# mandt-lab/shallow-ntc

Hardware: AMD Instinct MI355X
Metric: decode Mpixels/s + (bpp, PSNR) on Kodak, two_layer_syn (higher is better)
Workload: dtype f32

## Files before the change

include/sntc.h:

```cpp
#ifndef SNTC_H_
#define SNTC_H_

#include <stddef.h>
#include <stdint.h>

#ifdef __cplusplus
extern "C" {
#endif

#define SNTC_VERSION 100

enum {
  SNTC_OK = 0,
  SNTC_ERR_BAD_SHAPE = 1,
  SNTC_ERR_UNSUPPORTED = 2,
  SNTC_ERR_HIP = 3,
  SNTC_ERR_NONFINITE = 4,
  SNTC_ERR_NO_DEVICE = 5
};

const char* sntc_last_error(void);
int sntc_version(void);
int sntc_device_count(void);
int sntc_device_arch(int device, char* buf, size_t buflen);
// ... 80 lines not shown
int sntc_upsmall_plan_update(sntc_upsmall_plan* plan, const float* w, const float* bias, void* stream);
void sntc_upsmall_plan_destroy(sntc_upsmall_plan* plan);
int64_t sntc_upsmall_flops(const sntc_upsmall_plan* plan, int n, int h, int w);
int sntc_upsmall_forward(const sntc_upsmall_plan* plan, const float* x, int n, int h, int w, float* y, void* stream);
typedef struct sntc_syn_plan sntc_syn_plan;
typedef struct sntc_syn_batch {
  const float* y_hat;
  float* hidden;
  int32_t n, h, w;
  int32_t reserved;
} sntc_syn_batch;
int sntc_syn_supported(int k, int stride, int cin, int ch, int has_res);
int sntc_syn_plan_create(int k, int stride, int cin, int ch, int has_res, int act_kind, const float* w1, const float* b1,
                         const float* beta, const float* gamma, void* stream, sntc_syn_plan** plan);
int sntc_syn_plan_update(sntc_syn_plan* plan, const float* w1, const float* b1, const float* beta, const float* gamma, void* stream);
void sntc_syn_plan_destroy(sntc_syn_plan* plan);
int64_t sntc_syn_flops(const sntc_syn_plan* plan, int64_t latent_pixels);
int64_t sntc_syn_workspace_bytes(const sntc_syn_plan* plan);
int sntc_syn_forward(const sntc_syn_plan* plan, const sntc_syn_batch* batches, int nbatches, void* workspace, size_t workspace_bytes,
                     void* stream);
int sntc_syn_plan_set_workgroups(sntc_syn_plan* plan, int max_workgroups);
int sntc_syn_plan_units(const sntc_syn_plan* plan, int* out, int capacity);
int sntc_syn_describe(int k, int stride, int cin, int ch, int has_res, int* out, int capacity);
int sntc_syn_selfcheck(int k, int stride, int cin, int ch, int has_res, int h, int w, unsigned seed, double* max_err);
int sntc_conv_plan_set_tile(sntc_conv_plan* plan, int variant);
int sntc_conv_plan_set_schedule(sntc_conv_plan* plan, int flags);
int sntc_split3(const float* x, int64_t npix, int c, void* out, void* stream);
int sntc_dequant_split3(const int32_t* symbols, const float* hyper, int64_t npix, int c, void* out, float* y_hat,
                        void* stream);
int sntc_conv_status(int* flags, void* stream);
int sntc_conv_status_inject(int flags, void* stream);
int sntc_conv_set_stream_k(int enabled);
int sntc_conv_get_stream_k(void);
int sntc_conv_launch_info(const sntc_conv_plan* plan, int n, int h, int w, int* variant, int* nblocks);
int sntc_conv_launch_order(const sntc_conv_plan* plan, int n, int h, int w, int* column_major);
int64_t sntc_conv_tune_workspace_bytes(const sntc_conv_plan* plan, int n, int h, int w);
int sntc_conv_plan_tune(sntc_conv_plan* plan, const float* x, int n, int h, int w, float* y, const float* res,
                        const float* aux, void* workspace, size_t workspace_bytes, int reps, int* variant, int* stream_k,
                        void* stream);
int sntc_conv_plan_candidates(const sntc_conv_plan* plan, int n, int h, int w, int* variants, int* stream_k, int capacity);
int sntc_conv_plan_set_choice(sntc_conv_plan* plan, int n, int h, int w, int variant, int stream_k);
int sntc_conv_plan_clear_tuning(sntc_conv_plan* plan);
int sntc_conv_plan_drop_choice(sntc_conv_plan* plan, int n, int h, int w, int ncols);

int sntc_conv_columns_supported(const sntc_conv_plan* plan, int ncols);
int sntc_conv_forward_columns(const sntc_conv_plan* plan, const float* x, int n, int h, int w, float* y, const float* res,
                              const float* aux, void* workspace, size_t workspace_bytes, void* stream, int ncols);
int sntc_conv_forward_columns_dequant(const sntc_conv_plan* plan, const float* x, int n, int h, int w, int ncols,
                                      const int32_t* symbols, float* y_hat, void* workspace, size_t workspace_bytes, void* stream);
int64_t sntc_conv_columns_flops(const sntc_conv_plan* plan, int n, int h, int w, int ncols);
int64_t sntc_conv_columns_workspace_bytes(const sntc_conv_plan* plan, int n, int h, int w, int ncols);
int sntc_conv_columns_launch_info(const sntc_conv_plan* plan, int n, int h, int w, int ncols, int* variant, int* nblocks,
                                  int* column_major);
int64_t sntc_conv_columns_tune_workspace_bytes(const sntc_conv_plan* plan, int n, int h, int w, int ncols);
int sntc_conv_columns_tune(sntc_conv_plan* plan, const float* x, int n, int h, int w, int ncols, float* y, void* workspace,
                           size_t workspace_bytes, int reps, int* variant, int* stream_k, void* stream);
int sntc_conv_columns_candidates(const sntc_conv_plan* plan, int n, int h, int w, int ncols, int* variants, int* stream_k,
                                 int capacity);
int sntc_conv_columns_set_choice(sntc_conv_plan* plan, int n, int h, int w, int ncols, int variant, int stream_k);

int sntc_gdn_small(const float* x, int64_t npix, int c, const float* beta, const float* gamma,
                   int inverse, int alpha, int epsilon_is_half, float* y, void* stream);

int sntc_two_layer_tail(const float* t, int n, int hh, int wh, int ch, int has_res, int act_kind,
                        const float* beta, const float* gamma, const float* w2, const float* b2,
                        int k2, int s2, int cout, float* x_hat, void* stream);
// ... 198 lines not shown
```

shallow-ntc_amd/_capi.py:

```python
from __future__ import annotations

import ctypes as C
import os
from pathlib import Path

_PKG = Path(__file__).resolve().parent
LIB_PATH = Path(os.environ.get("SNTC_LIB", _PKG / "lib" / "libsntc_hip.so"))

OK, ERR_BAD_SHAPE, ERR_UNSUPPORTED, ERR_HIP, ERR_NONFINITE, ERR_NO_DEVICE = range(6)

CONV2D, CONV2D_TRANSPOSE, SIGNAL_DOWN, SIGNAL_UP = range(4)
ACT_NONE, ACT_RELU, ACT_LEAKY_RELU, ACT_SIGMOID = range(4)
PRO_NONE, PRO_ABS, PRO_SQUARE = range(3)
EPI_STORE, EPI_ADD, EPI_GATE, EPI_RES_DIV, EPI_RES_MUL, EPI_RES_DIV_SQRT, EPI_RES_MUL_SQRT, EPI_MASK_RELU, EPI_MASK_LEAKY = range(9)


class SntcError(RuntimeError):
    def __init__(self, code, msg):
        super().__init__(f"sntc error {code}: {msg}")
        self.code = code


class NonFiniteError(SntcError, ValueError):
    """Mirrors tf.debugging.check_numerics' InvalidArgumentError (reference mshyper/models.py:308-309,356)."""
# ... 37 lines not shown
    "sntc_resblock_forward": (C.c_int, [_P, _P, C.c_int, C.c_int, C.c_int, _P, _P]),
    "sntc_resblock_plan_set_workgroups": (C.c_int, [_P, C.c_int]),
    "sntc_upsmall_supported": (C.c_int, [C.c_int, C.c_int, C.c_int, C.c_int, C.c_int]),
    "sntc_upsmall_plan_create": (C.c_int, [C.c_int, C.c_int, C.c_int, C.c_int, C.c_int, _P, _P, _P, C.POINTER(_P)]),
    "sntc_upsmall_plan_update": (C.c_int, [_P, _P, _P, _P]),
    "sntc_upsmall_plan_destroy": (None, [_P]),
    "sntc_upsmall_flops": (C.c_int64, [_P, C.c_int, C.c_int, C.c_int]),
    "sntc_upsmall_forward": (C.c_int, [_P, _P, C.c_int, C.c_int, C.c_int, _P, _P]),
    "sntc_rgbconv_supported": (C.c_int, [C.c_int, C.c_int, C.c_int, C.c_int, C.c_int, C.c_int]),
    "sntc_rgbconv_plan_create": (C.c_int, [C.c_int, C.c_int, C.c_int, C.c_int, C.c_int, _P, _P, C.c_int, _P, C.POINTER(_P)]),
    "sntc_rgbconv_plan_update": (C.c_int, [_P, _P, _P, _P]),
    "sntc_rgbconv_plan_destroy": (None, [_P]),
    "sntc_rgbconv_flops": (C.c_int64, [_P, C.c_int, C.c_int, C.c_int]),
    "sntc_rgbconv_forward": (C.c_int, [_P, _P, C.c_int, C.c_int, C.c_int, _P, _P]),
    "sntc_rgbconv_plan_set_workgroups": (C.c_int, [_P, C.c_int]),
    "sntc_syn_supported": (C.c_int, [C.c_int, C.c_int, C.c_int, C.c_int, C.c_int]),
    "sntc_syn_plan_create": (C.c_int, [C.c_int, C.c_int, C.c_int, C.c_int, C.c_int, C.c_int, _P, _P, _P, _P, _P, C.POINTER(_P)]),
    "sntc_syn_plan_update": (C.c_int, [_P, _P, _P, _P, _P, _P]),
    "sntc_syn_plan_destroy": (None, [_P]),
    "sntc_syn_flops": (C.c_int64, [_P, C.c_int64]),
    "sntc_syn_workspace_bytes": (C.c_int64, [_P]),
    "sntc_syn_forward": (C.c_int, [_P, _P, C.c_int, _P, C.c_size_t, _P]),
    "sntc_syn_plan_set_workgroups": (C.c_int, [_P, C.c_int]),
    "sntc_syn_plan_units": (C.c_int, [_P, C.POINTER(C.c_int), C.c_int]),
    "sntc_syn_describe": (C.c_int, [C.c_int, C.c_int, C.c_int, C.c_int, C.c_int, C.POINTER(C.c_int), C.c_int]),
    "sntc_syn_selfcheck": (C.c_int, [C.c_int, C.c_int, C.c_int, C.c_int, C.c_int, C.c_int, C.c_int, C.c_uint, C.POINTER(C.c_double)]),
    "sntc_conv_plan_set_tile": (C.c_int, [C.c_void_p, C.c_int]),
    "sntc_conv_plan_set_schedule": (C.c_int, [C.c_void_p, C.c_int]),
    "sntc_split3": (C.c_int, [_P, C.c_int64, C.c_int, _P, _P]),
    "sntc_dequant_split3": (C.c_int, [_P, _P, C.c_int64, C.c_int, _P, _P, _P]),
    "sntc_conv_status": (C.c_int, [C.POINTER(C.c_int), _P]),
    "sntc_conv_status_inject": (C.c_int, [C.c_int, _P]),
    "sntc_conv_set_stream_k": (C.c_int, [C.c_int]),
    "sntc_conv_get_stream_k": (C.c_int, []),
    "sntc_conv_launch_info": (C.c_int, [_P, C.c_int, C.c_int, C.c_int, C.POINTER(C.c_int), C.POINTER(C.c_int)]),
    "sntc_conv_launch_order": (C.c_int, [_P, C.c_int, C.c_int, C.c_int, C.POINTER(C.c_int)]),
    "sntc_conv_tune_workspace_bytes": (C.c_int64, [_P, C.c_int, C.c_int, C.c_int]),
    "sntc_conv_plan_tune": (C.c_int, [_P, _P, C.c_int, C.c_int, C.c_int, _P, _P, _P, _P, C.c_size_t, C.c_int, C.POINTER(C.c_int),
                                      C.POINTER(C.c_int), _P]),
    "sntc_conv_plan_clear_tuning": (C.c_int, [_P]),
    "sntc_conv_plan_candidates": (C.c_int, [_P, C.c_int, C.c_int, C.c_int, C.POINTER(C.c_int), C.POINTER(C.c_int), C.c_int]),
    "sntc_conv_plan_set_choice": (C.c_int, [_P, C.c_int, C.c_int, C.c_int, C.c_int, C.c_int]),
    "sntc_conv_plan_drop_choice": (C.c_int, [_P, C.c_int, C.c_int, C.c_int, C.c_int]),
    "sntc_conv_columns_supported": (C.c_int, [_P, C.c_int]),
    "sntc_conv_forward_columns": (C.c_int, [_P, _P, C.c_int, C.c_int, C.c_int, _P, _P, _P, _P, C.c_size_t, _P, C.c_int]),
    "sntc_conv_forward_columns_dequant": (C.c_int, [_P, _P, C.c_int, C.c_int, C.c_int, C.c_int, _P, _P, _P, C.c_size_t, _P]),
    "sntc_conv_columns_flops": (C.c_int64, [_P, C.c_int, C.c_int, C.c_int, C.c_int]),
    "sntc_conv_columns_workspace_bytes": (C.c_int64, [_P, C.c_int, C.c_int, C.c_int, C.c_int]),
    "sntc_conv_columns_launch_info": (C.c_int, [_P, C.c_int, C.c_int, C.c_int, C.c_int, C.POINTER(C.c_int), C.POINTER(C.c_int),
                                                C.POINTER(C.c_int)]),
    "sntc_conv_columns_tune_workspace_bytes": (C.c_int64, [_P, C.c_int, C.c_int, C.c_int, C.c_int]),
    "sntc_conv_columns_tune": (C.c_int, [_P, _P, C.c_int, C.c_int, C.c_int, C.c_int, _P, _P, C.c_size_t, C.c_int, C.POINTER(C.c_int),
                                         C.POINTER(C.c_int), _P]),
    "sntc_conv_columns_candidates": (C.c_int, [_P, C.c_int, C.c_int, C.c_int, C.c_int, C.POINTER(C.c_int), C.POINTER(C.c_int), C.c_int]),
    "sntc_conv_columns_set_choice": (C.c_int, [_P, C.c_int, C.c_int, C.c_int, C.c_int, C.c_int, C.c_int]),
    "sntc_gdn_small": (C.c_int, [_P, C.c_int64, C.c_int, _P, _P, C.c_int, C.c_int, C.c_int, _P, _P]),
    "sntc_two_layer_tail": (C.c_int, [_P, C.c_int, C.c_int, C.c_int, C.c_int, C.c_int, C.c_int, _P, _P, _P, _P,
                                      C.c_int, C.c_int, C.c_int, _P, _P]),
    "sntc_two_layer_tail_pixels": (C.c_int, [_P, C.c_int, C.c_int, C.c_int, C.c_int, C.c_int, C.c_int, _P, _P, _P, _P,
                                             C.c_int, C.c_int, C.c_int, C.c_int, C.c_int, _P, _P, _P, _P]),
    "sntc_pad_reflect": (C.c_int, [_P, C.c_int, C.c_int, C.c_int, C.c_int, C.c_int, C.c_int, _P, _P]),
    "sntc_pad_zero": (C.c_int, [_P, C.c_int, C.c_int, C.c_int, C.c_int, C.c_int, C.c_int, C.c_int, C.c_int, _P, _P]),
    "sntc_crop": (C.c_int, [_P, C.c_int, C.c_int, C.c_int, C.c_int, C.c_int, C.c_int, _P, _P]),
    "sntc_depth_to_space": (C.c_int, [_P, C.c_int, C.c_int, C.c_int, C.c_int, C.c_int, _P, _P]),
    "sntc_concat_channels": (C.c_int, [_P, C.c_int, _P, C.c_int, C.c_int64, _P, _P]),
    "sntc_pixels_sse": (C.c_int, [_P, _P, C.c_int, C.c_int, C.c_int, C.c_int, C.c_int, C.c_int, _P, _P, _P]),
# ... 149 lines not shown
```

shallow-ntc_amd/csrc/conv_plan.hip:

```cpp
#include <algorithm>
#include <cstdio>
#include <cstdlib>
#include <array>
#include <atomic>
#include <map>
#include <mutex>
#include <cstdlib>
#include <vector>
#include "sntc_internal.h"
#include "gg_tap_rules.h"

namespace sntc {

struct PackDesc {
  const float* w;
  float* wp;
  const int* taps;
  const unsigned* cols;
  int T, Cin, Cout, K, Ncol, kw, s, pt, pl, phase_mode, slab_major, out_major, bf3, rowpack;
};

__device__ __forceinline__ void pack_element(const PackDesc& d, size_t idx) {
  const int col = (int)(idx / d.K);
  const int k = (int)(idx - (size_t)col * d.K);
// ... 743 lines not shown
  const int64_t x_bytes = (int64_t)n * h * w * d.cin * (p->s3 ? 6 : 4);
  if (M > 0x7fffffffLL || x_bytes >= (1LL << 31))
    return fail(SNTC_ERR_BAD_SHAPE, "sntc_conv_forward: input tensor must be < 2 GiB (32-bit buffer offsets); split the batch");
  if (p2 && M * p2->d.cout >= (1LL << 32)) return fail(SNTC_ERR_BAD_SHAPE, "sntc_conv_forward_fused: output too large; split the batch");
  const Sched sc = force ? schedule(p, g, n, false, force, ncols) : plan_schedule(p, g, n, h, w, p2 != nullptr, ncols);
  if (!sc.inst) return fail(SNTC_ERR_UNSUPPORTED, "sntc_conv_forward: no compiled instance for this plan and tile variant");
  const int64_t ws_floats = workspace_floats(p, M, sc, ncols);
  if (ws_floats > 0 && (!workspace || workspace_bytes < (size_t)ws_floats * 4))
    return fail(SNTC_ERR_BAD_SHAPE, "sntc_conv_forward: this call needs sntc_conv_workspace_bytes() of workspace "
                                    "(split-K slabs / stream-K hand-off)");
  const GGInstance& inst = *sc.inst;
  const Work wk = work_of(p, inst, M, ncols);
  if (sc.sk && wk.units != sc.units) return fail(SNTC_ERR_HIP, "sntc_conv_forward: schedule and launch disagree about the work units");
  GGArgs a{};
  a.ksplit = sc.ksplit;
  a.slab = static_cast<float*>(workspace);
  a.x = x; a.y = y; a.bias = p->bias; a.res = res; a.aux = aux;
  a.x_bytes = (unsigned)x_bytes;
  a.N = n; a.H = h; a.W = w; a.Cin = d.cin;
  a.Qh = g.Qh; a.Qw = g.Qw; a.M = (int)M;
  a.Ho = g.Ho; a.Wo = g.Wo; a.Cout = ncols > 0 ? ncols : d.cout;
  a.sA = g.sA; a.tstep = g.tstep; a.offy = g.offy; a.offx = g.offx; a.sO = g.sO;
  a.act = d.act; a.epi = epilogue; a.pro = d.prologue;
  a.ntm = wk.ntm;
  a.ngroups = p->ngroups;
  if (p2) { a.w2f = p2->w2f; a.bias2 = p2->bias; a.Cout2 = p2->d.cout; }
  a.status = gg_status_word();
  if (!a.status) return fail(SNTC_ERR_HIP, "sntc_conv_forward: the device tables of the current device are not initialised");
  a.sk = sc.sk ? 1 : 0;
  a.nworkers = sc.workers;
  a.units = wk.units;
  if (sc.sk) {
    a.sk_slab = static_cast<float*>(workspace);
    a.sk_flags = reinterpret_cast<int*>(a.sk_slab + (size_t)sc.workers * inst.slab_floats);
    a.slab = nullptr;
    if (int zrc = zero_async(a.sk_flags, sizeof(int) * sc.workers, (hipStream_t)stream)) return zrc;
  }
  int nb = 0;
  size_t slab_off = 0;
  for (int gi = 0; gi < p->ngroups; ++gi) {
    GGGroup& G = a.g[gi];
    G.wp = p->g[gi].wp; G.taps = p->g[gi].taps; G.cols = reinterpret_cast<const int*>(p->g[gi].cols);
    G.T = p->g[gi].T; G.K = p->g[gi].K; G.Ncol = launch_cols(p, gi, ncols); G.tw = p->g[gi].tw;
    G.ntn = wk.ntn[gi];
    G.steps = G.K / kStage;
    G.blk0 = nb;
    G.tile0 = wk.tile0[gi];
    G.unit0 = wk.unit0[gi];
    nb += G.ntn * a.ntm * sc.ksplit;
    G.slab_off = slab_off;
    G.q0y = p->g[gi].q0y; G.q0x = p->g[gi].q0x;
    slab_off += (size_t)sc.ksplit * M * G.Ncol;
  }
  a.tps = wk.tps;
  a.ups = (int)wk.ups;
  if (p->s3) a.order = p->dma == 0 ? 0 : 1;
  rc = gg_launch(inst, a, sc.sk ? sc.workers : nb, (hipStream_t)stream);
  if (rc || sc.sk || sc.ksplit <= 1) return rc;
  return gg_reduce_launch(a, (hipStream_t)stream);
}

extern "C" int sntc_conv_forward(const sntc_conv_plan* p, const float* x, int n, int h, int w, float* y,
                                 const float* res, const float* aux, void* workspace, size_t workspace_bytes,
                                 void* stream) {
  return conv_forward_impl(p, nullptr, x, n, h, w, y, res, aux, workspace, workspace_bytes, stream);
}

static void tune_candidates(const sntc_conv_plan* p, const Geo& g, int n, std::vector<std::pair<TuneChoice, Sched>>* out, int ncols = 0) {
  for (int v = 1; v <= kMaxVariant; ++v) {
// ... 176 lines not shown
  if (!p) return fail(SNTC_ERR_BAD_SHAPE, "sntc_conv_plan_clear_tuning: null plan");
  std::lock_guard<std::mutex> lk(p->tune_mu);
  p->tuned.clear();
  return SNTC_OK;
}

static const char* fused_pair_error(const sntc_conv_plan* p, const sntc_conv_plan* p2) {
  if (!p || !p2) return "null plan";
  const sntc_conv_desc& a = p->d;
  if (p->up || p2->up || p->bf3 || p2->bf3) return "forward convolutions in fp32 only";
  if (!p->vec || a.cout != 96 || a.stride != 1 || a.prologue != SNTC_PRO_NONE || a.epilogue != SNTC_EPI_STORE || p->ngroups != 1)
    return "first plan: stride-1 convolution with Cin % 16 == 0 and 96 output channels, plain store";
  if (!fusable_second(p2) || !p2->w2f) return "second plan: 1x1 convolution 96 -> 192 without activation";
  return nullptr;
}

extern "C" int sntc_conv_fusable(const sntc_conv_plan* p, const sntc_conv_plan* p2) { return fused_pair_error(p, p2) ? 0 : 1; }

extern "C" int64_t sntc_conv_fused_workspace_bytes(const sntc_conv_plan* p, int n, int h, int w) {
  if (!p) return 0;
  Geo g;
  if (geometry(p, h, w, &g)) return 0;
  return 4 * workspace_floats(p, (int64_t)n * g.Qh * g.Qw, schedule(p, g, n, true));
}

extern "C" int sntc_conv_forward_fused(const sntc_conv_plan* p, const sntc_conv_plan* p2, const float* x, int n, int h, int w, float* y,
                                       const float* res, const float* aux, void* workspace, size_t workspace_bytes,
                                       void* stream) {
  if (const char* why = fused_pair_error(p, p2)) return fail(SNTC_ERR_UNSUPPORTED, why);
  return conv_forward_impl(p, p2, x, n, h, w, y, res, aux, workspace, workspace_bytes, stream);
}

extern "C" int sntc_conv_set_stream_k(int enabled) {
  g_stream_k_enabled.store(enabled ? 1 : 0, std::memory_order_relaxed);
  return SNTC_OK;
}

extern "C" int sntc_conv_get_stream_k(void) { return g_stream_k_enabled.load(std::memory_order_relaxed); }

__global__ void status_exchange_kernel(int* word, int* out) { *out = atomicExch(word, 0); }
__global__ void status_or_kernel(int* word, int flags) { atomicOr(word, flags); }

extern "C" int sntc_conv_status(int* flags, void* stream) {
  if (!flags) return fail(SNTC_ERR_BAD_SHAPE, "sntc_conv_status: null argument");
  int rc = gg_init();
  if (rc) return rc;
  int* word = gg_status_word();
  hipStream_t s = (hipStream_t)stream;
  hipLaunchKernelGGL(status_exchange_kernel, dim3(1), dim3(1), 0, s, word, word + 1);
  SNTC_HIP(hipGetLastError());
  SNTC_HIP(hipMemcpyAsync(flags, word + 1, sizeof(int), hipMemcpyDeviceToHost, s));
  SNTC_HIP(hipStreamSynchronize(s));
  return SNTC_OK;
}

extern "C" int sntc_conv_status_inject(int flags, void* stream) {
  int rc = gg_init();
  if (rc) return rc;
  hipLaunchKernelGGL(status_or_kernel, dim3(1), dim3(1), 0, (hipStream_t)stream, gg_status_word(), flags);
  SNTC_HIP(hipGetLastError());
  return SNTC_OK;
}
```

shallow-ntc_amd/csrc/gather_gemm.hip:

```cpp
#include "gather_gemm_kernel.h"

namespace sntc {

#define SNTC_GG_DECL_VEC(TM, TN, WM, WN) extern template __global__ void gg_kernel<TM, TN, WM, WN, true, false>(const GGArgs);
#define SNTC_GG_DECL_PRO(TM, TN, WM, WN)                                                   \
  extern template __global__ void gg_kernel<TM, TN, WM, WN, true, true>(const GGArgs);    \
  extern template __global__ void gg_kernel<TM, TN, WM, WN, false, true>(const GGArgs);
#define SNTC_GG_DECL_DMA(TM, TN, WM, WN) extern template __global__ void gg_kernel<TM, TN, WM, WN, true, false, false, true>(const GGArgs);
SNTC_GG_SHAPES(SNTC_GG_DECL_VEC)
SNTC_GG_SHAPES(SNTC_GG_DECL_PRO)
SNTC_GG_DMA_SHAPES(SNTC_GG_DECL_DMA)
extern template __global__ void gg_kernel<1, 1, 2, 2, true, false, false, true, kDeepRing>(const GGArgs);
extern template __global__ void gg_kernel<1, 3, 4, 1, true, false, false, false, 0, true>(const GGArgs);
extern template __global__ void gg_kernel<2, 2, 2, 2, true, false, false, false, 0, false, true>(const GGArgs);
extern template __global__ void gg_kernel<1, 2, 4, 1, true, false, true>(const GGArgs);
extern template __global__ void gg_kernel<1, 4, 4, 1, true, false, true>(const GGArgs);

__global__ void __launch_bounds__(256) gg_reduce_kernel(const GGArgs a) {
  const GGGroup G = a.g[blockIdx.y];
  const size_t total = (size_t)a.M * G.Ncol;
  const int per = a.Qh * a.Qw;
  for (size_t i = blockIdx.x * (size_t)blockDim.x + threadIdx.x; i < total; i += (size_t)gridDim.x * blockDim.x) {
    const int m = (int)(i / G.Ncol);
    const int col = (int)(i - (size_t)m * G.Ncol);
    float v = 0.0f;
    for (int sp = 0; sp < a.ksplit; ++sp) v += a.slab[G.slab_off + (size_t)sp * total + i];
    const unsigned ce = G.cols[col];
    const int ch = ce & 0xffff;
    const int n = m / per;
    const int rem = m - n * per;
    const int qy = rem / a.Qw + G.q0y, qx = rem - (rem / a.Qw) * a.Qw + G.q0x;
    const int oy = qy * a.sO + (int)((ce >> 24) & 0xff) - 128;
    const int ox = qx * a.sO + (int)((ce >> 16) & 0xff) - 128;
// ... 39 lines not shown
    GG_LOADERS(1, 1, 1, 4, 1), GG_LOADERS(2, 1, 2, 4, 1), GG_LOADERS(3, 1, 3, 4, 1), GG_LOADERS(4, 1, 4, 4, 1), GG_LOADERS(5, 1, 5, 4, 1),
    GG_LOADERS(6, 1, 6, 4, 1), GG_LOADERS(7, 1, 7, 4, 1), GG_LOADERS(8, 1, 1, 2, 2), GG_LOADERS(9, 2, 2, 2, 2), GG_LOADERS(10, 2, 4, 4, 1),
    GG_DMA(1, 1, 1, 4, 1), GG_DMA(2, 1, 2, 4, 1), GG_DMA(3, 1, 3, 4, 1), GG_DMA(4, 1, 4, 4, 1), GG_DMA(5, 1, 5, 4, 1),
    GG_DMA(8, 1, 1, 2, 2), GG_DMA(9, 2, 2, 2, 2),
    GG(8, kLoadVec, kStageDeep, kFormPlain, 1, 1, 2, 2, true, false, false, true, kDeepRing),
    GG(3, kLoadVec, kStageRing, kFormFuse2, 1, 3, 4, 1, true, false, false, false, 0, true),
    GG(9, kLoadVec, kStageRing, kFormColm, 2, 2, 2, 2, true, false, false, false, 0, false, true),
    GG(2, kLoadVec, kStageRing, kFormBf3, 1, 2, 4, 1, true, false, true),
    GG(4, kLoadVec, kStageRing, kFormBf3, 1, 4, 4, 1, true, false, true),
    BF3P(11, 4, kFormPresplit), BF3P(11, 4, kFormPresplitHalo), BF3P(12, 2, kFormPresplit), BF3P(12, 2, kFormPresplitHalo),
    BF3P(13, 3, kFormPresplit), BF3P(13, 3, kFormPresplitHalo),
};
#undef GG
#undef GG_LOADERS
#undef GG_DMA
#undef BF3P
constexpr int kNumInstances = sizeof(kInstances) / sizeof(kInstances[0]);

const GGInstance* gg_find(int variant, GGLoad load, GGStage stage, GGForm form) {
  for (const GGInstance& r : kInstances)
    if (r.variant == variant && r.load == load && r.stage == stage && r.form == form) return &r;
  return nullptr;
}

static bool presplit(const GGInstance& r) { return r.form == kFormPresplit || r.form == kFormPresplitHalo; }

constexpr int kMaxDevices = 16;
struct DeviceTables {
  std::once_flag once;
  int rc = SNTC_OK;
  int num_cus = 0;
  int resident[kNumInstances] = {};
  int* status = nullptr;
};
static DeviceTables g_dev[kMaxDevices];

static int fill_tables(DeviceTables& T, int dev) {
  hipDeviceProp_t prop;
  SNTC_HIP(hipGetDeviceProperties(&prop, dev));
  T.num_cus = prop.multiProcessorCount;
  for (int i = 0; i < kNumInstances; ++i) {
    const GGInstance& r = kInstances[i];
    SNTC_HIP(hipFuncSetAttribute(r.fn, hipFuncAttributeMaxDynamicSharedMemorySize, (int)r.lds));
    if (presplit(r)) {
      T.resident[i] = T.num_cus;
      continue;
    }
    int per_cu = 0;
    SNTC_HIP(hipOccupancyMaxActiveBlocksPerMultiprocessor(&per_cu, r.fn, r.threads, r.lds));
    per_cu = std::max(1, std::min({per_cu, 8, (int)(163840 / r.lds)}));
    T.resident[i] = per_cu * T.num_cus;
  }
  SNTC_HIP(hipMalloc(&T.status, 2 * sizeof(int)));
  SNTC_HIP(hipMemset(T.status, 0, 2 * sizeof(int)));
  return SNTC_OK;
}

static DeviceTables* current_tables() {
  int dev = 0;
  if (hipGetDevice(&dev) != hipSuccess || dev < 0 || dev >= kMaxDevices) return nullptr;
  DeviceTables& T = g_dev[dev];
  std::call_once(T.once, [&] { T.rc = fill_tables(T, dev); });
  return T.rc == SNTC_OK ? &T : nullptr;
}

int gg_init() {
  int dev = 0;
  SNTC_HIP(hipGetDevice(&dev));
  if (dev < 0 || dev >= kMaxDevices) return fail(SNTC_ERR_UNSUPPORTED, "device index beyond the residency tables");
  DeviceTables& T = g_dev[dev];
  std::call_once(T.once, [&] { T.rc = fill_tables(T, dev); });
  return T.rc;
}

int gg_resident(const GGInstance& inst) {
  const DeviceTables* T = current_tables();
  return T ? T->resident[&inst - kInstances] : 0;
}

int gg_num_cus() {
  const DeviceTables* T = current_tables();
  return T ? T->num_cus : 0;
}

int* gg_status_word() {
  const DeviceTables* T = current_tables();
  return T ? T->status : nullptr;
}

int gg_launch(const GGInstance& inst, const GGArgs& args, int nblocks, hipStream_t stream) {
  GGArgs a = args;
  a.dma = inst.stage;
  a.bf3 = inst.form == kFormBf3 || presplit(inst) ? 1 : 0;
  a.halo = inst.form == kFormPresplitHalo ? 1 : 0;
  if (!presplit(inst)) a.order = inst.form == kFormColm ? 0 : 1;
#ifdef SNTC_DIAG
  if (const char* e = getenv("SNTC_GG_DBG")) a.dbg = atoi(e);
#endif
  void* params[] = {&a};
  hipError_t e = hipLaunchKernel(inst.fn, dim3(nblocks), dim3(inst.threads), params, inst.lds, stream);
  if (e != hipSuccess) return hip_fail(e, "gather-GEMM launch");
  return SNTC_OK;
}

}
```

shallow-ntc_amd/csrc/gg_pieces.h:

```cpp
#pragma once

#if defined(__HIPCC__)
#include "sntc_internal.h"
#define SNTC_PIECE_FN __host__ __device__ __forceinline__
#define SNTC_PIECE_UNROLL _Pragma("unroll")
#else
#define SNTC_PIECE_FN inline
#define SNTC_PIECE_UNROLL
#endif

namespace sntc {

constexpr int kPieceGroups = 4;

struct Piece {
  int gi, mt, nt, k0, k1;
  int consume;
  int publish;
  int split;
};

enum { kOrderRuntime = -1, kOrderColumn = 0, kOrderStrip = 1 };
template <int ORDER, class A>
SNTC_PIECE_FN bool strip_major(const A& a) { return ORDER == kOrderRuntime ? a.order == kOrderStrip : ORDER == kOrderStrip; }
// ... 146 lines not shown
__device__ __forceinline__ KArgs& fresh_args() {
  KArgs* kp = (KArgs*)__builtin_amdgcn_kernarg_segment_ptr();
  asm volatile("" : "+s"(kp));
  return *kp;
}

template <int BM, int NT>
__device__ __forceinline__ void write_rinfo(KArgs& a, const Piece& p, int4* rinfo, int tid) {
  const int mbase = p.mt * BM;
  const int q0y = a.g[p.gi].q0y, q0x = a.g[p.gi].q0x;
  for (int r = tid; r < BM; r += NT) {
    const int m = mbase + r;
    int4 ri = make_int4(0, 0, 0, 0);
    if (m < a.M) {
      const int per = a.Qh * a.Qw;
      const int n = m / per;
      const int rem = m - n * per;
      const int qy = rem / a.Qw;
      ri = make_int4(n, qy + q0y, rem - qy * a.Qw + q0x, 1);
    }
    rinfo[r] = ri;
  }
}

template <int TM, int TN, int NT>
__device__ __forceinline__ __amdgpu_buffer_rsrc_t sk_slab_of(float* sk_slab, int worker) {
  return __builtin_amdgcn_make_buffer_rsrc(sk_slab + (size_t)worker * (TM * TN * 16 * NT), 0, TM * TN * 16 * NT * 4, 0x00020000);
}

template <int TM, int TN, int NT, class A>
__device__ __forceinline__ void sk_consume(const A& a, int worker, int tid, f32x16 (&acc)[TM][TN]) {
  if (tid == 0) {
    int spins = 0;
    while (__hip_atomic_load(a.sk_flags + worker, __ATOMIC_RELAXED, __HIP_MEMORY_SCOPE_AGENT) == 0) {
      __builtin_amdgcn_s_sleep(8);
      if (++spins > kSpinLimit) {
        __hip_atomic_fetch_or(fresh_args().status, 1, __ATOMIC_RELAXED, __HIP_MEMORY_SCOPE_AGENT);
        break;
      }
    }
    __builtin_amdgcn_fence(__ATOMIC_ACQUIRE, "agent");
    asm volatile("s_waitcnt vmcnt(0)" ::: "memory");
  }
  __syncthreads();
  const __amdgpu_buffer_rsrc_t sr = sk_slab_of<TM, TN, NT>(a.sk_slab, worker);
#pragma unroll
  for (int i = 0; i < TM; ++i)
#pragma unroll
    for (int j = 0; j < TN; ++j)
#pragma unroll
      for (int q = 0; q < 4; ++q) {
        const u32x4 v = __builtin_amdgcn_raw_buffer_load_b128(sr, tid * 16, ((i * TN + j) * 4 + q) * NT * 16, 0);
        const f32x4 f = __builtin_bit_cast(f32x4, v);
        acc[i][j][4 * q] = f[0]; acc[i][j][4 * q + 1] = f[1]; acc[i][j][4 * q + 2] = f[2]; acc[i][j][4 * q + 3] = f[3];
      }
}

template <int TM, int TN, int NT, class A>
__device__ __forceinline__ void sk_publish(const A& a, int wl, int tid, const f32x16 (&acc)[TM][TN]) {
  const __amdgpu_buffer_rsrc_t sr = sk_slab_of<TM, TN, NT>(a.sk_slab, wl);
#pragma unroll
  for (int i = 0; i < TM; ++i)
#pragma unroll
    for (int j = 0; j < TN; ++j)
#pragma unroll
      for (int q = 0; q < 4; ++q) {
        const f32x4 v = {acc[i][j][4 * q], acc[i][j][4 * q + 1], acc[i][j][4 * q + 2], acc[i][j][4 * q + 3]};
        __builtin_amdgcn_raw_buffer_store_b128(__builtin_bit_cast(u32x4, v), sr, tid * 16, ((i * TN + j) * 4 + q) * NT * 16, 0);
      }
  asm volatile("s_waitcnt vmcnt(0)" ::: "memory");
  __syncthreads();
  if (tid == 0) {
    __builtin_amdgcn_fence(__ATOMIC_RELEASE, "agent");
    asm volatile("s_waitcnt vmcnt(0)" ::: "memory");
    __hip_atomic_store(a.sk_flags + wl, 1, __ATOMIC_RELAXED, __HIP_MEMORY_SCOPE_AGENT);
// ... 6 lines not shown
```

shallow-ntc_amd/csrc/sntc_internal.h:

```cpp
#pragma once
#include <hip/hip_runtime.h>
#include <stdint.h>
#include <string>
#include "../../include/sntc.h"

namespace sntc {

void set_error(const std::string& msg);
int fail(int code, const std::string& msg);
int hip_fail(hipError_t e, const char* what);
int zero_async(void* p, size_t bytes, hipStream_t stream);

#define SNTC_HIP(expr)                                         \
  do {                                                         \
    hipError_t _e = (expr);                                    \
    if (_e != hipSuccess) return ::sntc::hip_fail(_e, #expr);  \
  } while (0)

constexpr int kMaxGroups = 4;

#ifdef SNTC_DIAG
#define SNTC_DBG(a, bit) (((a).dbg & (bit)) != 0)
#else
#define SNTC_DBG(a, bit) false
#endif

struct GGGroup {
  const float* wp;
  const int* taps;
  const int* cols;
  int T;
  int tw;
  int K;
  int Ncol;
  int ntn;
  int blk0;
  size_t slab_off;
  int q0y, q0x;
  int steps;
  int tile0;
  long long unit0;
};

struct GGArgs {
// ... 92 lines not shown
```

shallow-ntc_amd/csrc/syn_fused.hip:

```cpp
#include <algorithm>
#include <cmath>
#include <cstdio>
#include <cstdlib>
#include <cstring>
#include <mutex>
#include <vector>
#include "sntc_internal.h"

#include "rb_common.h"

namespace sntc {
namespace syn {

using rb::buf_load;
using rb::buf_store;
using rb::kOOB;

constexpr int kNT = 3;
constexpr int kRows = 32 * kNT;
constexpr int kUnit = kRows * 16;
constexpr int kRing = 8;
constexpr int kLead = 5;
constexpr int kPSlots = 3;
constexpr int kPPMax = 512;
constexpr int kPStride = (kPPMax + 1) * 16;
constexpr int kTileM = 256;
constexpr int kMaxSynGroups = 4;
constexpr int kMaxSlots = 8;

struct SynUnit {
  int ns;
  unsigned sl0, sl1;
  int step0;
  unsigned ph[kMaxSlots];
  int cost;
  unsigned pm;
  int pad[2];
};
static_assert(sizeof(SynUnit) == 64, "SynUnit is read as 16 dwords");

// ... 138 lines not shown
        float* dst = patch + pslot * kPStride + (wave + 8 * i) * 256;
        __builtin_amdgcn_raw_ptr_buffer_load_lds(xs, (lds_void*)dst, 16, (int)pvoff[i], cc * 64, 0, 0);
      }
  };

  __syncthreads();
  int item = blockIdx.x;
  if (item >= a.nitems) return;
  Item I{};
  decode(item, &I);
  setup_loader(I);
  struct UnitHot {
    int ns, step0;
    unsigned sl0, sl1, pm;
  };
  auto load_unit = [&](int u, UnitHot* U) {
    const SynUnit* up = syn_args().units + u;
    U->ns = up->ns; U->step0 = up->step0; U->sl0 = up->sl0; U->sl1 = up->sl1; U->pm = up->pm;
  };
  auto shift_of = [&](const UnitHot& U, int j) { return (int)(((j < 8 ? U.sl0 >> (4 * j) : U.sl1 >> (4 * (j - 8)))) & 15u); };
  const int nslab = a.nslab;
  UnitHot U;
  load_unit(I.u, &U);
  auto prologue = [&](const UnitHot& U) {
    const int T = nslab * U.ns;
    dma_patch(0, 0);
    if (nslab > 1) dma_patch(1, 1);
#pragma unroll
    for (int u = 0; u < kLead; ++u)
      if (u < T) dma_w(U.step0 + u, u);
  };
  prologue(U);
  int fetched = 0;
  if (tid == 0) fetched = atomicAdd(syn_args().queue, 1) + (int)gridDim.x;
  int islot = 0;

  while (true) {
    const int HW = I.H * I.W;
    const int m = I.m0 + 32 * wave + l31;
    const bool pvalid = m < HW;
    const int qy = m / I.W, qx = m - qy * I.W;
    unsigned vmask = 0;
#pragma unroll
    for (int si = 0; si < 9; ++si) {
      const int dy = 1 - si / 3, dx = 1 - si % 3;
      if (pvalid && (unsigned)(qy + dy) < (unsigned)I.H && (unsigned)(qx + dx) < (unsigned)I.W) vmask |= 1u << si;
    }
    const int lanepp = 32 * wave + l31 + I.W + 1;
    const int zoff = kPPMax * 16;
    auto read_p = [&](int ps, int si, int g) -> f32x4 {
      const int q3 = si / 3;
      const int pp = lanepp + (1 - q3) * I.W + 1 - (si - 3 * q3);
      const int off = pp * 16 + ((((2 * g + h) ^ ((pp >> 2) & 3))) << 2);
      const int sel = -(int)((vmask >> si) & 1u);
      return *reinterpret_cast<const f32x4*>(patch + (ps * kPStride + ((off & sel) | (zoff & ~sel))));
    };

    const int ns = U.ns;
    const int T = nslab * ns;

    asm volatile("s_waitcnt vmcnt(0) lgkmcnt(0)" ::: "memory");
    if (tid == 0) sh_item[islot] = fetched;
    __builtin_amdgcn_s_barrier();
    __builtin_amdgcn_sched_barrier(0);

    f32x16 acc[kNT];
#pragma unroll
    for (int jt = 0; jt < kNT; ++jt)
#pragma unroll
      for (int e = 0; e < 16; ++e) acc[jt][e] = 0.0f;

    f32x4 Fw0[kNT], Fw1[kNT], FwN[kNT];
    f32x4 Fp0, Fp1, FpN;
    int cc = 0, j = 0, ps = 0;
    int si = shift_of(U, 0);

    auto step = [&](int t, auto MASKEDc) {
      constexpr bool MASKED = decltype(MASKEDc)::value;
      int jn = j + 1, ccn = cc, psn = ps;
      if (jn == ns) {
        jn = 0;
        ccn = cc + 1;
        psn = ps == kPSlots - 1 ? 0 : ps + 1;
      }
      const int sin = shift_of(U, jn);
      const bool third = !MASKED || !((U.pm >> j) & 1u);
      if (j == 0 && cc + 2 < nslab && !SNTC_DBG(a, 2)) dma_patch(cc + 2, ps == 0 ? 2 : ps - 1);
      const bool wdma = t + kLead < T && !SNTC_DBG(a, 4);
      if (wdma) dma_w(U.step0 + t + kLead, (t + kLead) & (kRing - 1));
      __builtin_amdgcn_sched_barrier(0);
      read_w(Fw1, t & (kRing - 1), 1);
      Fp1 = read_p(ps, si, 1);
      if (!SNTC_DBG(a, 8)) {
#pragma unroll
        for (int e = 0; e < 4; ++e)
// ... 133 lines not shown
              asm volatile("s_waitcnt vmcnt(0) lgkmcnt(0)" ::: "memory");
            }
            if (!SNTC_DBG(a, 16)) __builtin_amdgcn_s_barrier();
            __builtin_amdgcn_sched_barrier(0);
          }
        });
        psl = psn;
      }
    };
    using N1 = std::integral_constant<int, 1>;
    using N2 = std::integral_constant<int, 2>;
    using N4 = std::integral_constant<int, 4>;
    const bool generic = SNTC_DBG(a, 32);
    if (!generic && ns == 4 && U.pm == 0) kloop(N4{}, std::integral_constant<unsigned, 0>{});
    else if (!generic && ns == 4 && U.pm == 0xcu) kloop(N4{}, std::integral_constant<unsigned, 0xc>{});
    else if (!generic && ns == 4 && U.pm == 0xau) kloop(N4{}, std::integral_constant<unsigned, 0xa>{});
    else if (!generic && ns == 2 && U.pm == 0) kloop(N2{}, std::integral_constant<unsigned, 0>{});
    else if (!generic && ns == 1 && U.pm == 0) kloop(N1{}, std::integral_constant<unsigned, 0>{});
    else if (U.pm == 0) {
      read_w(Fw0, 0, 0);
      Fp0 = read_p(0, si, 0);
#pragma unroll 1
      for (int t = 0; t < T; ++t) step(t, std::integral_constant<bool, false>{});
    } else {
      read_w(Fw0, 0, 0);
      Fp0 = read_p(0, si, 0);
#pragma unroll 1
      for (int t = 0; t < T; ++t) step(t, std::integral_constant<bool, true>{});
    }

    const int item_next = __builtin_amdgcn_readfirstlane(sh_item[islot]);
    islot ^= 1;
    const Item Icur = I;
    const bool more = item_next < syn_args().nitems;
    if (more) {
      decode(item_next, &I);
      setup_loader(I);
      load_unit(I.u, &U);
      prologue(U);
      if (tid == 0) fetched = atomicAdd(syn_args().queue, 1) + (int)gridDim.x;
    }
    __builtin_amdgcn_sched_barrier(0);

    if (!SNTC_DBG(a, 1)) {
      SynKArgs& a = syn_args();
      const SynUnit* up = a.units + Icur.u;
      const int Wo = Icur.W * a.s;
      const __amdgpu_buffer_rsrc_t vs = __builtin_amdgcn_make_buffer_rsrc(
          a.g[Icur.gi].v + (size_t)Icur.n * HW * (a.s * a.s) * CH, 0, HW * (a.s * a.s) * CH * 4, 0x00020000);
      const float* bias = tab;
      const float* beta = tab + CP;
      const float* gamma = tab + CP + CH;
      typedef float f32x2 __attribute__((ext_vector_type(2)));
      const int act = a.act_kind;
#pragma unroll
      for (int sl = 0; sl < SPH; ++sl) {
        float tv[CP];
#pragma unroll
        for (int c = 0; c < CP; ++c) {
          const int vi = sl * CP + c;
          tv[c] = acc[vi >> 4][vi & 15] + bias[c];
        }
        float o[CH];
        if (act == 1 || act == 2) {
          float av[CH];
#pragma unroll
          for (int ic = 0; ic < CH; ++ic) av[ic] = fabsf(tv[ic]);
          f32x2 nrm[CH / 2];
#pragma unroll
          for (int jp = 0; jp < CH / 2; ++jp) nrm[jp] = *reinterpret_cast<const f32x2*>(beta + 2 * jp);
#pragma unroll
          for (int ic = 0; ic < CH; ++ic)
#pragma unroll
// ... 314 lines not shown
}

extern "C" int64_t sntc_syn_workspace_bytes(const sntc_syn_plan* p) { return p ? 256 : -1; }

extern "C" int sntc_syn_forward(const sntc_syn_plan* p, const sntc_syn_batch* batches, int nbatches, void* workspace, size_t workspace_bytes,
                                void* stream) {
  if (!p || !batches || !workspace) return fail(SNTC_ERR_BAD_SHAPE, "sntc_syn_forward: null argument");
  if (nbatches < 1 || nbatches > kMaxSynGroups) return fail(SNTC_ERR_BAD_SHAPE, "sntc_syn_forward: 1 .. 4 batches per call");
  if (workspace_bytes < 256) return fail(SNTC_ERR_BAD_SHAPE, "sntc_syn_forward: workspace smaller than sntc_syn_workspace_bytes()");
  const HostPlan& P = p->P;
  SynArgs a{};
  int64_t tiles = 0;
  int ng = 0;
  for (int i = 0; i < nbatches; ++i) {
    const sntc_syn_batch& b = batches[i];
    if (b.n < 0 || b.h < 0 || b.w < 0) return fail(SNTC_ERR_BAD_SHAPE, "sntc_syn_forward: negative size");
    if (b.n == 0 || b.h == 0 || b.w == 0) continue;
    if (!b.y_hat || !b.hidden) return fail(SNTC_ERR_BAD_SHAPE, "sntc_syn_forward: null tensor");
    if (kTileM + 2 * b.w + 2 > kPPMax) return fail(SNTC_ERR_UNSUPPORTED, "sntc_syn_forward: latent rows wider than 127 pixels");
    const int64_t hw = (int64_t)b.h * b.w;
    if (hw * P.G.cin * 4 >= (1LL << 31) || hw * P.G.s * P.G.s * P.ch * 4 >= (1LL << 31))
      return fail(SNTC_ERR_BAD_SHAPE, "sntc_syn_forward: one image's tensor of 2 GiB or more");
    SynGroup& g = a.g[ng++];
    g.x = b.y_hat; g.v = b.hidden; g.n = b.n; g.h = b.h; g.w = b.w;
    g.tile0 = (int)tiles;
    g.tpi = (int)((hw + kTileM - 1) / kTileM);
    tiles += (int64_t)b.n * g.tpi;
    if (tiles * (int64_t)P.units.size() >= (1LL << 30)) return fail(SNTC_ERR_BAD_SHAPE, "sntc_syn_forward: too many work items");
  }
  if (ng == 0) return SNTC_OK;
  int cus = 0;
  if (int rc = syn_init(&cus)) return rc;
  a.wpack = p->wpack; a.units = p->units; a.tables = p->tables;
  a.queue = reinterpret_cast<int*>(workspace);
  a.wbytes = (unsigned)((size_t)P.total_steps * kUnit * 4);
  a.nunits = (int)P.units.size(); a.ntiles = (int)tiles; a.nitems = a.nunits * a.ntiles;
  a.cin = P.G.cin; a.nslab = P.nslab; a.s = P.G.s; a.act_kind = p->act_kind;
  a.ngroups = ng;
#ifdef SNTC_DIAG
  if (const char* e = getenv("SNTC_SYN_DBG")) a.dbg = atoi(e);
#endif
  hipStream_t s = (hipStream_t)stream;
  if (int zrc = zero_async(workspace, 64, s)) return zrc;
  const int grid = std::min<int64_t>(a.nitems, p->max_workgroups > 0 ? p->max_workgroups : cus);
  const void* fn = nullptr;
  size_t lds = 0;
  const int cp = P.G.cp;
  if (cp == 12 && !P.has_res) { fn = reinterpret_cast<const void*>(&syn_kernel<12, false>); lds = SynCfg<12, false>::LDS; }
  else if (cp == 24 && !P.has_res) { fn = reinterpret_cast<const void*>(&syn_kernel<24, false>); lds = SynCfg<24, false>::LDS; }
  else if (cp == 24 && P.has_res) { fn = reinterpret_cast<const void*>(&syn_kernel<24, true>); lds = SynCfg<24, true>::LDS; }
  else if (cp == 48 && !P.has_res) { fn = reinterpret_cast<const void*>(&syn_kernel<48, false>); lds = SynCfg<48, false>::LDS; }
  else if (cp == 48 && P.has_res) { fn = reinterpret_cast<const void*>(&syn_kernel<48, true>); lds = SynCfg<48, true>::LDS; }
  else return fail(SNTC_ERR_UNSUPPORTED, "sntc_syn_forward: no kernel for this width");
  void* params[] = {&a};
  hipError_t e = hipLaunchKernel(fn, dim3(grid), dim3(512), params, lds, s);
  if (e != hipSuccess) return hip_fail(e, "synthesis launch");
  return SNTC_OK;
}

extern "C" int sntc_syn_selfcheck(int k, int stride, int cin, int ch, int has_res, int h, int w, unsigned seed, double* max_err) {
  if (!max_err) return fail(SNTC_ERR_BAD_SHAPE, "sntc_syn_selfcheck: null argument");
  HostPlan P;
  if (int rc = build_host_plan(k, stride, cin, ch, has_res ? 1 : 0, &P)) return rc;
  if (h < 1 || w < 1 || kTileM + 2 * w + 2 > kPPMax) return fail(SNTC_ERR_BAD_SHAPE, "sntc_syn_selfcheck: bad image size");
  const SynGeom G = P.G;
  const int cp = G.cp, s = G.s;
  unsigned st = seed * 2654435761u + 12345u;
  auto rnd = [&]() { st = st * 1664525u + 1013904223u; return (double)((st >> 8) & 0xffff) / 32768.0 - 1.0; };
  std::vector<float> wk((size_t)k * k * cp * cin), x((size_t)h * w * cin);
  for (auto& v : wk) v = (float)rnd();
  for (auto& v : x) v = (float)rnd();
  const int Ho = h * s, Wo = w * s;
  std::vector<double> ref((size_t)Ho * Wo * cp, 0.0), got((size_t)Ho * Wo * cp, 0.0);
  std::vector<int> hits((size_t)Ho * Wo, 0);
  for (int iy = 0; iy < h; ++iy)
    for (int ix = 0; ix < w; ++ix)
// ... 78 lines not shown
```

Baseline: 4192.

## Use persistent self-resetting sync lanes to skip per-launch zeroing memsets

Adds a per-device arena of synchronisation words, with one lane per stream. The work-queue counter and stream-K flags live in these lanes instead of in the caller's workspace. Kernels now reset their own counters: the last ticket holder clears the queue, and consumers clear the flags they observed. This removes the zero_async memset launch before every synthesis and stream-K conv launch. In exchange it adds host-side stream-capture checks, a mutex, dirty-state recovery after a spin timeout, and the risk of stale counters if a launch aborts.

Result: no change. 4200 (median of 6 runs) (+0.2%).

```diff
diff --git a/include/sntc.h b/include/sntc.h
--- a/include/sntc.h
+++ b/include/sntc.h
@@ -136,6 +136,7 @@
 int sntc_conv_status_inject(int flags, void* stream);
 int sntc_conv_set_stream_k(int enabled);
 int sntc_conv_get_stream_k(void);
+int sntc_sync_lane_nonzero(void* stream, int* count);
 int sntc_conv_launch_info(const sntc_conv_plan* plan, int n, int h, int w, int* variant, int* nblocks);
 int sntc_conv_launch_order(const sntc_conv_plan* plan, int n, int h, int w, int* column_major);
 int64_t sntc_conv_tune_workspace_bytes(const sntc_conv_plan* plan, int n, int h, int w);
diff --git a/shallow-ntc_amd/_capi.py b/shallow-ntc_amd/_capi.py
--- a/shallow-ntc_amd/_capi.py
+++ b/shallow-ntc_amd/_capi.py
@@ -93,6 +93,7 @@
     "sntc_conv_status": (C.c_int, [C.POINTER(C.c_int), _P]),
     "sntc_conv_status_inject": (C.c_int, [C.c_int, _P]),
     "sntc_conv_set_stream_k": (C.c_int, [C.c_int]),
+    "sntc_sync_lane_nonzero": (C.c_int, [_P, C.POINTER(C.c_int)]),
     "sntc_conv_get_stream_k": (C.c_int, []),
     "sntc_conv_launch_info": (C.c_int, [_P, C.c_int, C.c_int, C.c_int, C.POINTER(C.c_int), C.POINTER(C.c_int)]),
     "sntc_conv_launch_order": (C.c_int, [_P, C.c_int, C.c_int, C.c_int, C.POINTER(C.c_int)]),
diff --git a/shallow-ntc_amd/csrc/conv_plan.hip b/shallow-ntc_amd/csrc/conv_plan.hip
--- a/shallow-ntc_amd/csrc/conv_plan.hip
+++ b/shallow-ntc_amd/csrc/conv_plan.hip
@@ -799,9 +799,11 @@
   a.units = wk.units;
   if (sc.sk) {
     a.sk_slab = static_cast<float*>(workspace);
-    a.sk_flags = reinterpret_cast<int*>(a.sk_slab + (size_t)sc.workers * inst.slab_floats);
     a.slab = nullptr;
-    if (int zrc = zero_async(a.sk_flags, sizeof(int) * sc.workers, (hipStream_t)stream)) return zrc;
+    SyncWords sw;
+    if (int zrc = sync_words((hipStream_t)stream, reinterpret_cast<int*>(a.sk_slab + (size_t)sc.workers * inst.slab_floats), sc.workers, &sw))
+      return zrc;
+    a.sk_flags = sw.flags;
   }
   int nb = 0;
   size_t slab_off = 0;
@@ -1044,6 +1046,8 @@
 }
 
 extern "C" int sntc_conv_set_stream_k(int enabled) {
+  if (enabled)
+    if (int rc = sync_lanes_clean()) return rc;
   g_stream_k_enabled.store(enabled ? 1 : 0, std::memory_order_relaxed);
   return SNTC_OK;
 }
@@ -1063,6 +1067,10 @@
   SNTC_HIP(hipGetLastError());
   SNTC_HIP(hipMemcpyAsync(flags, word + 1, sizeof(int), hipMemcpyDeviceToHost, s));
   SNTC_HIP(hipStreamSynchronize(s));
+  if (*flags != 0) {
+    sync_lanes_mark_dirty();
+    return sync_lanes_clean();
+  }
   return SNTC_OK;
 }
 
diff --git a/shallow-ntc_amd/csrc/gather_gemm.hip b/shallow-ntc_amd/csrc/gather_gemm.hip
--- a/shallow-ntc_amd/csrc/gather_gemm.hip
+++ b/shallow-ntc_amd/csrc/gather_gemm.hip
@@ -1,4 +1,6 @@
+#include <mutex>
 #include "gather_gemm_kernel.h"
+#include "sync_lanes.h"
 
 namespace sntc {
 
@@ -104,6 +106,9 @@
   int num_cus = 0;
   int resident[kNumInstances] = {};
   int* status = nullptr;
+  std::mutex lanes_mutex;
+  SyncLaneMap lanes;
+  int* arena = nullptr;
 };
 static DeviceTables g_dev[kMaxDevices];
 
@@ -125,6 +130,9 @@
   }
   SNTC_HIP(hipMalloc(&T.status, 2 * sizeof(int)));
   SNTC_HIP(hipMemset(T.status, 0, 2 * sizeof(int)));
+  SNTC_HIP(hipMalloc(&T.arena, sizeof(int) * kSyncLanes * kSyncLaneWords));
+  SNTC_HIP(hipMemset(T.arena, 0, sizeof(int) * kSyncLanes * kSyncLaneWords));
+  SNTC_HIP(hipDeviceSynchronize());
   return SNTC_OK;
 }
 
@@ -160,6 +168,79 @@
   return T ? T->status : nullptr;
 }
 
+#ifdef SNTC_DIAG
+static int sync_dbg() {
+  const char* e = getenv("SNTC_SYNC_DBG");
+  return e ? atoi(e) : 0;
+}
+#endif
+
+int sync_words(hipStream_t stream, int* fallback, int fallback_words, SyncWords* out) {
+  DeviceTables* T = current_tables();
+  if (!T) return fail(SNTC_ERR_HIP, "the device tables of the current device are not initialised");
+  int lane = kNoLane;
+  bool use_lane = fallback_words <= kSyncFlagWords;
+#ifdef SNTC_DIAG
+  if (sync_dbg() & 1) use_lane = false;
+#endif
+  if (use_lane && stream) {
+    hipStreamCaptureStatus cap = hipStreamCaptureStatusNone;
+    if (hipStreamIsCapturing(stream, &cap) != hipSuccess) {
+      (void)hipGetLastError();
+      use_lane = false;
+    } else if (cap != hipStreamCaptureStatusNone) {
+      use_lane = false;
+    }
+  }
+  if (use_lane) {
+    std::lock_guard<std::mutex> lock(T->lanes_mutex);
+    lane = T->lanes.acquire(stream);
+  }
+  if (lane != kNoLane) {
+    out->queue = T->arena + (size_t)lane * kSyncLaneWords;
+    out->flags = out->queue + kSyncQueueWords;
+    return SNTC_OK;
+  }
+  out->queue = out->flags = fallback;
+  if (int rc = zero_async(fallback, sizeof(int) * (size_t)fallback_words, stream)) return rc;
+#ifdef SNTC_DIAG
+  if (sync_dbg() & 2) return zero_async(fallback, sizeof(int) * (size_t)fallback_words, stream);
+#endif
+  return SNTC_OK;
+}
+
+void sync_lanes_mark_dirty() {
+  DeviceTables* T = current_tables();
+  if (!T) return;
+  std::lock_guard<std::mutex> lock(T->lanes_mutex);
+  T->lanes.dirty = true;
+}
+
+int sync_lanes_clean() {
+  int rc = SNTC_OK;
+  for (int dev = 0; dev < kMaxDevices; ++dev) {
+    DeviceTables& T = g_dev[dev];
+    {
+      std::lock_guard<std::mutex> lock(T.lanes_mutex);
+      if (!T.lanes.dirty) continue;
+    }
+    int cur = 0;
+    hipError_t e = hipGetDevice(&cur);
+    if (e == hipSuccess && cur != dev) e = hipSetDevice(dev);
+    if (e == hipSuccess) e = hipDeviceSynchronize();
+    if (e == hipSuccess) e = hipMemset(T.arena, 0, sizeof(int) * kSyncLanes * kSyncLaneWords);
+    if (e == hipSuccess) e = hipDeviceSynchronize();
+    if (cur != dev) (void)hipSetDevice(cur);
+    if (e != hipSuccess) {
+      rc = hip_fail(e, "zeroing the synchronisation arena");
+      continue;
+    }
+    std::lock_guard<std::mutex> lock(T.lanes_mutex);
+    T.lanes.dirty = false;
+  }
+  return rc;
+}
+
 int gg_launch(const GGInstance& inst, const GGArgs& args, int nblocks, hipStream_t stream) {
   GGArgs a = args;
   a.dma = inst.stage;
@@ -176,3 +257,26 @@
 }
 
 }
+
+extern "C" int sntc_sync_lane_nonzero(void* stream, int* count) {
+  using namespace sntc;
+  if (!count) return fail(SNTC_ERR_BAD_SHAPE, "sntc_sync_lane_nonzero: null argument");
+  int rc = gg_init();
+  if (rc) return rc;
+  DeviceTables* T = current_tables();
+  if (!T) return fail(SNTC_ERR_HIP, "sntc_sync_lane_nonzero: the device tables of the current device are not initialised");
+  int lane;
+  {
+    std::lock_guard<std::mutex> lock(T->lanes_mutex);
+    lane = T->lanes.find(stream);
+  }
+  *count = -1;
+  if (lane == kNoLane) return SNTC_OK;
+  static thread_local int words[kSyncLaneWords];
+  SNTC_HIP(hipDeviceSynchronize());
+  SNTC_HIP(hipMemcpy(words, T->arena + (size_t)lane * kSyncLaneWords, sizeof(words), hipMemcpyDeviceToHost));
+  int n = 0;
+  for (int i = 0; i < kSyncLaneWords; ++i) n += words[i] != 0;
+  *count = n;
+  return SNTC_OK;
+}
diff --git a/shallow-ntc_amd/csrc/gg_pieces.h b/shallow-ntc_amd/csrc/gg_pieces.h
--- a/shallow-ntc_amd/csrc/gg_pieces.h
+++ b/shallow-ntc_amd/csrc/gg_pieces.h
@@ -202,15 +202,18 @@
 __device__ __forceinline__ void sk_consume(const A& a, int worker, int tid, f32x16 (&acc)[TM][TN]) {
   if (tid == 0) {
     int spins = 0;
+    bool seen = true;
     while (__hip_atomic_load(a.sk_flags + worker, __ATOMIC_RELAXED, __HIP_MEMORY_SCOPE_AGENT) == 0) {
       __builtin_amdgcn_s_sleep(8);
       if (++spins > kSpinLimit) {
         __hip_atomic_fetch_or(fresh_args().status, 1, __ATOMIC_RELAXED, __HIP_MEMORY_SCOPE_AGENT);
+        seen = false;
         break;
       }
     }
     __builtin_amdgcn_fence(__ATOMIC_ACQUIRE, "agent");
     asm volatile("s_waitcnt vmcnt(0)" ::: "memory");
+    if (seen) __hip_atomic_store(a.sk_flags + worker, 0, __ATOMIC_RELAXED, __HIP_MEMORY_SCOPE_AGENT);
   }
   __syncthreads();
   const __amdgpu_buffer_rsrc_t sr = sk_slab_of<TM, TN, NT>(a.sk_slab, worker);
diff --git a/shallow-ntc_amd/csrc/sntc_internal.h b/shallow-ntc_amd/csrc/sntc_internal.h
--- a/shallow-ntc_amd/csrc/sntc_internal.h
+++ b/shallow-ntc_amd/csrc/sntc_internal.h
@@ -10,6 +10,14 @@
 int fail(int code, const std::string& msg);
 int hip_fail(hipError_t e, const char* what);
 int zero_async(void* p, size_t bytes, hipStream_t stream);
+
+struct SyncWords {
+  int* queue;
+  int* flags;
+};
+int sync_words(hipStream_t stream, int* fallback, int fallback_words, SyncWords* out);
+void sync_lanes_mark_dirty();
+int sync_lanes_clean();
 
 #define SNTC_HIP(expr)                                         \
   do {                                                         \
diff --git a/shallow-ntc_amd/csrc/syn_fused.hip b/shallow-ntc_amd/csrc/syn_fused.hip
--- a/shallow-ntc_amd/csrc/syn_fused.hip
+++ b/shallow-ntc_amd/csrc/syn_fused.hip
@@ -6,6 +6,7 @@
 #include <mutex>
 #include <vector>
 #include "sntc_internal.h"
+#include "sync_lanes.h"
 
 #include "rb_common.h"
 
@@ -210,7 +211,7 @@
   };
   prologue(U);
   int fetched = 0;
-  if (tid == 0) fetched = atomicAdd(syn_args().queue, 1) + (int)gridDim.x;
+  if (tid == 0) fetched = syn_ticket_item(atomicAdd(syn_args().queue, 1), (int)gridDim.x);
   int islot = 0;
 
   while (true) {
@@ -238,7 +239,12 @@
     const int T = nslab * ns;
 
     asm volatile("s_waitcnt vmcnt(0) lgkmcnt(0)" ::: "memory");
-    if (tid == 0) sh_item[islot] = fetched;
+    if (tid == 0) {
+      sh_item[islot] = fetched;
+      SynKArgs& a = syn_args();
+      if (fetched == syn_ticket_item(syn_total_tickets(a.nitems, (int)gridDim.x) - 1, (int)gridDim.x))
+        __hip_atomic_store(a.queue, 0, __ATOMIC_RELAXED, __HIP_MEMORY_SCOPE_AGENT);
+    }
     __builtin_amdgcn_s_barrier();
     __builtin_amdgcn_sched_barrier(0);
 
@@ -438,13 +444,13 @@
     const int item_next = __builtin_amdgcn_readfirstlane(sh_item[islot]);
     islot ^= 1;
     const Item Icur = I;
-    const bool more = item_next < syn_args().nitems;
+    const bool more = syn_draws_after(item_next, syn_args().nitems);
     if (more) {
       decode(item_next, &I);
       setup_loader(I);
       load_unit(I.u, &U);
       prologue(U);
-      if (tid == 0) fetched = atomicAdd(syn_args().queue, 1) + (int)gridDim.x;
+      if (tid == 0) fetched = syn_ticket_item(atomicAdd(syn_args().queue, 1), (int)gridDim.x);
     }
     __builtin_amdgcn_sched_barrier(0);
 
@@ -825,7 +831,6 @@
   int cus = 0;
   if (int rc = syn_init(&cus)) return rc;
   a.wpack = p->wpack; a.units = p->units; a.tables = p->tables;
-  a.queue = reinterpret_cast<int*>(workspace);
   a.wbytes = (unsigned)((size_t)P.total_steps * kUnit * 4);
   a.nunits = (int)P.units.size(); a.ntiles = (int)tiles; a.nitems = a.nunits * a.ntiles;
   a.cin = P.G.cin; a.nslab = P.nslab; a.s = P.G.s; a.act_kind = p->act_kind;
@@ -834,7 +839,9 @@
   if (const char* e = getenv("SNTC_SYN_DBG")) a.dbg = atoi(e);
 #endif
   hipStream_t s = (hipStream_t)stream;
-  if (int zrc = zero_async(workspace, 64, s)) return zrc;
+  SyncWords sw;
+  if (int zrc = sync_words(s, reinterpret_cast<int*>(workspace), kSyncQueueWords, &sw)) return zrc;
+  a.queue = sw.queue;
   const int grid = std::min<int64_t>(a.nitems, p->max_workgroups > 0 ? p->max_workgroups : cus);
   const void* fn = nullptr;
   size_t lds = 0;
diff --git a/shallow-ntc_amd/csrc/sync_lanes.h b/shallow-ntc_amd/csrc/sync_lanes.h
--- /dev/null
+++ b/shallow-ntc_amd/csrc/sync_lanes.h
@@ -0,0 +1,46 @@
+#pragma once
+
+#if defined(__HIPCC__)
+#define SNTC_LANE_FN __host__ __device__ __forceinline__
+#else
+#define SNTC_LANE_FN inline
+#endif
+
+namespace sntc {
+
+constexpr int kSyncLanes = 64;
+constexpr int kSyncQueueWords = 16;
+constexpr int kSyncFlagWords = 2048;
+constexpr int kSyncLaneWords = kSyncQueueWords + kSyncFlagWords;
+constexpr int kNoLane = -1;
+
+struct SyncLaneMap {
+  const void* key[kSyncLanes] = {};
+  int used = 0;
+  bool dirty = false;
+
+  int find(const void* stream) const {
+    for (int i = 0; i < used; ++i)
+      if (key[i] == stream) return i;
+    return kNoLane;
+  }
+  int acquire(const void* stream) {
+    if (dirty) return kNoLane;
+    const int i = find(stream);
+    if (i != kNoLane) return i;
+    if (used == kSyncLanes) return kNoLane;
+    key[used] = stream;
+    return used++;
+  }
+};
+
+SNTC_LANE_FN int syn_ticket_item(int ticket, int grid) { return ticket + grid; }
+SNTC_LANE_FN bool syn_draws_after(int item, int nitems) { return item < nitems; }
+SNTC_LANE_FN int syn_tickets_drawn(int b, int nitems, int in_range) { return b < nitems ? 1 + in_range : 0; }
+SNTC_LANE_FN int syn_total_tickets(int nitems, int grid) {
+  const int first = grid < nitems ? grid : nitems;
+  const int in_range = nitems > grid ? nitems - grid : 0;
+  return syn_tickets_drawn(0, nitems, 0) * first + in_range;
+}
+
+}
```
